# CITlabRostock/citlab-article-separation-new

Measured on AMD Instinct MI355X. Metric: newspaper pages/sec (ARU-Net seg + GNN relation) at 3000x4500 px, higher is better.
Workload: dtype f32s

## Files before the change

citlab-article-separation-new_amd/csrc/res8ws_kernels.h:

```cpp
#pragma once
#include "res8w_kernels.h"
#include "split_kernels.h"

namespace asep {

struct Res8WSProb {
    const float* skip;
    const float* dec;
    const float* img;
    const float* stats;
    float* out;
    float* pool;
    int H, W;
    int n_strips;
    int band;
    int y_end;
    int tile_begin;
};
struct Res8WSArgs {
    Res8WSProb p[MAXP];
    int nprob;
    const float* b1;
    const u32x4* w1s;
    const float* w1f;
    const u32x4* ws;
    const float* bias;
    XcdMap xm;
};

__device__ __forceinline__ void r8ws_mm6(const u32x4 (&w)[3], const u32x4 (&xa)[3], const u32x4 (&xb)[3], f32x4& ca, f32x4& cb) {
    ca = mfma_bf16_k32(w[2], xa[0], ca); cb = mfma_bf16_k32(w[2], xb[0], cb);
    ca = mfma_bf16_k32(w[0], xa[2], ca); cb = mfma_bf16_k32(w[0], xb[2], cb);
    ca = mfma_bf16_k32(w[1], xa[1], ca); cb = mfma_bf16_k32(w[1], xb[1], cb);
    ca = mfma_bf16_k32(w[1], xa[0], ca); cb = mfma_bf16_k32(w[1], xb[0], cb);
    ca = mfma_bf16_k32(w[0], xa[1], ca); cb = mfma_bf16_k32(w[0], xb[1], cb);
    ca = mfma_bf16_k32(w[0], xa[0], ca); cb = mfma_bf16_k32(w[0], xb[0], cb);
}
__device__ __forceinline__ void r8ws_split4(f32x4 v, u32x2& h, u32x2& m, u32x2& l) {
    unsigned h0, m0, l0, h1, m1, l1;
    split3_pair(v.x, v.y, h0, m0, l0);
    split3_pair(v.z, v.w, h1, m1, l1);
    h = u32x2{h0, h1}; m = u32x2{m0, m1}; l = u32x2{l0, l1};
}

template <bool UP>
__global__ __launch_bounds__(64, 1) void res8ws_kernel(const Res8WSArgs a) {
    constexpr int TW = R8W_TW;
    constexpr int W0 = TW + 6, W1 = TW + 4, W2 = TW + 2;
    constexpr int NR = 4, NT = 16;
    constexpr int PL0 = W0 * 16, PL1 = W1 * 16, PL2 = W2 * 16;
    constexpr int IMB = UP ? 0 : 4 * 32 * 4;
    constexpr int R0_OFF = IMB, R1_OFF = R0_OFF + NR * 3 * PL0, R2_OFF = R1_OFF + NR * 3 * PL1, TC_OFF = R2_OFF + NR * 3 * PL2,
                  TRASH = TC_OFF + NT * TW * 32, LDSB = TRASH + 16;
    static_assert(LDSB <= 30 * 1024, "four waves per CU with room to spare");
    __shared__ __attribute__((aligned(16))) unsigned char lds[LDSB];

    const int lane = threadIdx.x;
    const int j = lane & 15, kk = lane >> 4, e = kk >> 1, ch = (kk & 1) * 4;
    const int isB = kk & 1;
    const int c = 2 * j + e;
    const int item = sched_tile(a.xm);
    if (item < 0) return;
    const int pi = prob_of_tile(a, item);
    const Res8WSProb& P = a.p[pi];
    const int li = item - P.tile_begin;
    const int bi = li / P.n_strips, si = li - bi * P.n_strips;
    const int x0 = R8W_X0 + TW * si;
    const int Ya = R8W_Y0 + bi * P.band;
    const int nb = min(P.band, P.y_end - Ya);
    const int W = P.W;

    constexpr int NF1 = UP ? 18 : 0, NFW = 27;
    u32x4 wf[NFW], w1[UP ? NF1 : 1];
    {
        const u32x4* wl = a.ws + lane;
#pragma unroll
        for (int i = 0; i < NFW; ++i) asm volatile("global_load_dwordx4 %0, %1, off" : "=a"(wf[i]) : "v"(wl + i * 64) : "memory");
        if constexpr (UP) {
            const u32x4* w1l = a.w1s + lane;
#pragma unroll
            for (int i = 0; i < NF1; ++i) asm volatile("global_load_dwordx4 %0, %1, off" : "=a"(w1[i]) : "v"(w1l + i * 64) : "memory");
        }
        asm volatile("s_waitcnt vmcnt(0)" ::: "memory");
#pragma unroll
        for (int i = 0; i < NFW; ++i) asm volatile("" : "+a"(wf[i]));
        if constexpr (UP) {
#pragma unroll
            for (int i = 0; i < NF1; ++i) asm volatile("" : "+a"(w1[i]));
        }
    }
    auto wpart = [&](int s, int ky, u32x4 (&o)[3]) {
#pragma unroll
        for (int p = 0; p < 3; ++p) o[p] = wf[(s * 3 + ky) * 3 + p];
    };
    const f32x4 bias1 = *reinterpret_cast<const f32x4*>(a.b1 + ch);
    f32x4 biasw[3];
#pragma unroll
    for (int t = 0; t < 3; ++t) biasw[t] = *reinterpret_cast<const f32x4*>(a.bias + 8 * t + ch);

    const int gxw = min(x0 - 4 + 2 * j + kk, W - 1);
    const float* __restrict__ skp = P.skip;
    const float* __restrict__ dcp = P.dec;
    auto in_row = [&](const float* __restrict__ src, int gy, f32x4& lo, f32x4& hi) {
        const float* q = src + ((size_t)gy * (size_t)W + (size_t)gxw) * 8;
        lo = *reinterpret_cast<const f32x4*>(q);
        hi = *reinterpret_cast<const f32x4*>(q + 4);
    };
    float mean = 0.f, inv = 1.f;
    if constexpr (!UP) {
        if (P.stats) { mean = P.stats[0]; inv = P.stats[1]; }
    }
    const float* __restrict__ imp = P.img;
    const size_t ioff0 = (size_t)(Ya - 4 + (lane >> 5)) * (size_t)W + (size_t)(x0 - 4 + (lane & 31));
    auto iload = [&](int p) { return imp[ioff0 + (size_t)p * 2 * (size_t)W]; };
    float* const iring = reinterpret_cast<float*>(lds);
    auto istore = [&](float v, int p) { iring[(p & 1) * 64 + lane] = (v - mean) * inv; };
    float w1v[UP ? 1 : 36];
    if constexpr (!UP) {
#pragma unroll
        for (int t = 0; t < 9; ++t)
#pragma unroll
            for (int o = 0; o < 4; ++o) w1v[t * 4 + o] = a.w1f[t * 8 + ch + o];
    }

    const int p_last = nb / 2 + 3;
    u32x4 cin[2][2][3] = {};
    f32x4 nxt[2][2][2];
    float inx = 0.f;
    if constexpr (UP) {
#pragma unroll
        for (int r = 0; r < 2; ++r) {
            f32x4 lo, hi;
            in_row(skp, Ya - 4 + r, lo, hi);
            split3_x8(lo, hi, cin[r][0][0], cin[r][0][1], cin[r][0][2]);
            in_row(dcp, Ya - 4 + r, lo, hi);
            split3_x8(lo, hi, cin[r][1][0], cin[r][1][1], cin[r][1][2]);
            in_row(skp, Ya - 2 + r, nxt[r][0][0], nxt[r][0][1]);
            in_row(dcp, Ya - 2 + r, nxt[r][1][0], nxt[r][1][1]);
        }
    } else {
        istore(iload(0), 0);
        inx = iload(1);
    }

    const int lcol = r8w_swz(2 * j + kk) * 16;
    auto whole = [&](u32x2 pa, u32x2 pb) {
        const auto s0 = __builtin_amdgcn_permlane16_swap(pa.x, pb.x, false, false);
        const auto s1 = __builtin_amdgcn_permlane16_swap(pa.y, pb.y, false, false);
        return u32x4{s0[0], s1[0], s0[1], s1[1]};
    };
    const int cs = r8w_swz(c) * 16;
    const bool v0 = j < W0 / 2, v1 = j < W1 / 2, v2 = j < W2 / 2;
    const bool tvalid = c >= 3 && c < 3 + TW;
    const int tcol = (tvalid ? c - 3 : 0) * 32 + ch * 4;
    const int trd = min(c, TW - 1) * 32 + ch * 4;
    const bool ost = j < TW / 2;
    float* __restrict__ const outp = P.out;
    float* __restrict__ const poolp = P.pool;
    const size_t Wp = (size_t)((W + 1) >> 1);

    auto store_parts = [&](f32x4 ra, f32x4 rb, int roff, int pl, bool valid, int rowa, int rowb) {
        u32x2 ha, ma, la, hb, mb, lb;
        r8ws_split4(relu4i(ra), ha, ma, la);
        r8ws_split4(relu4i(rb), hb, mb, lb);
        const u32x4 ph = whole(ha, hb), pm = whole(ma, mb), pl_ = whole(la, lb);
        const int rr = isB ? rowb : rowa;
        const int base = valid ? roff + rr * 3 * pl + cs : TRASH;
        const int step = valid ? pl : 0;
        *reinterpret_cast<u32x4*>(lds + base) = ph;
        *reinterpret_cast<u32x4*>(lds + base + step) = pm;
        *reinterpret_cast<u32x4*>(lds + base + 2 * step) = pl_;
    };
    auto ring_read = [&](int roff, int pl, int rr, u32x4 (&o)[3]) {
#pragma unroll
        for (int p = 0; p < 3; ++p) o[p] = *reinterpret_cast<const u32x4*>(lds + roff + (rr * 3 + p) * pl + lcol);
    };

    const int K = nb / 2 + 6;
#pragma unroll 1
    for (int k = 0; k < K; ++k) {
        const int i4 = (2 * k) & (NR - 1), i16 = (2 * k) & (NT - 1);
        const bool do_c1 = k < nb / 2 + 3, do_s1 = k >= 2 && k < nb / 2 + 4, do_s2 = k >= 4 && k < nb / 2 + 5, do_s3 = k >= 6;

        if (do_s3) {
            u32x4 q[4][3];
#pragma unroll
            for (int r = 0; r < 4; ++r) ring_read(R2_OFF, PL2, (i4 + r - 9) & (NR - 1), q[r]);
            const f32x4 t0 = *reinterpret_cast<const f32x4*>(lds + TC_OFF + ((i16 - 8) & (NT - 1)) * TW * 32 + trd);
            const f32x4 t1 = *reinterpret_cast<const f32x4*>(lds + TC_OFF + ((i16 - 7) & (NT - 1)) * TW * 32 + trd);
            f32x4 va = biasw[2], vb = biasw[2];
#pragma unroll
            for (int ky = 0; ky < 3; ++ky) {
                u32x4 w[3];
                wpart(2, ky, w);
                r8ws_mm6(w, q[ky], q[ky + 1], va, vb);
            }
            va = relu4i(va + t0);
            vb = relu4i(vb + t1);
            const int oy = Ya - 12 + 2 * k;
            if (ost) {
                float* o = outp + ((size_t)oy * (size_t)W + (size_t)(x0 + c)) * 8 + ch;
                *reinterpret_cast<f32x4*>(o) = va;
                *reinterpret_cast<f32x4*>(o + (size_t)W * 8) = vb;
            }
            if constexpr (!UP) {
                if (poolp) {
                    const f32x4 mv = f32x4{fmaxf(va.x, vb.x), fmaxf(va.y, vb.y), fmaxf(va.z, vb.z), fmaxf(va.w, vb.w)};
                    float pm[4];
#pragma unroll
                    for (int i = 0; i < 4; ++i) {
                        const unsigned u = __float_as_uint(mv[i]);
                        const auto s = __builtin_amdgcn_permlane32_swap(u, u, false, false);
                        pm[i] = fmaxf(__uint_as_float(s[0]), __uint_as_float(s[1]));
                    }
                    if (ost && e == 0) {
                        float* po = poolp + ((size_t)(oy >> 1) * Wp + (size_t)((x0 >> 1) + j)) * 8 + ch;
                        *reinterpret_cast<f32x4*>(po) = f32x4{pm[0], pm[1], pm[2], pm[3]};
                    }
                }
            }
        }
        if (do_s2) {
            u32x4 q[4][3];
#pragma unroll
            for (int r = 0; r < 4; ++r) ring_read(R1_OFF, PL1, (i4 + r - 6) & (NR - 1), q[r]);
            f32x4 ra = biasw[1], rb = biasw[1];
#pragma unroll
            for (int ky = 0; ky < 3; ++ky) {
                u32x4 w[3];
                wpart(1, ky, w);
                r8ws_mm6(w, q[ky], q[ky + 1], ra, rb);
            }
            store_parts(ra, rb, R2_OFF, PL2, v2, (i4 - 5) & (NR - 1), (i4 - 4) & (NR - 1));
        }
        if (do_s1) {
            u32x4 q[4][3];
#pragma unroll
            for (int r = 0; r < 4; ++r) ring_read(R0_OFF, PL0, (i4 + r - 3) & (NR - 1), q[r]);
            f32x4 ra = biasw[0], rb = biasw[0];
#pragma unroll
            for (int ky = 0; ky < 3; ++ky) {
                u32x4 w[3];
                wpart(0, ky, w);
                r8ws_mm6(w, q[ky], q[ky + 1], ra, rb);
            }
            store_parts(ra, rb, R1_OFF, PL1, v1, (i4 - 2) & (NR - 1), (i4 - 1) & (NR - 1));
        }
        if (do_c1) {
            f32x4 ra = bias1, rb = bias1;
            if constexpr (UP) {
                u32x4 x2[2][2][3];
#pragma unroll
                for (int r = 0; r < 2; ++r)
#pragma unroll
                    for (int s = 0; s < 2; ++s) split3_x8(nxt[r][s][0], nxt[r][s][1], x2[r][s][0], x2[r][s][1], x2[r][s][2]);
                if (k + 2 <= p_last) {
#pragma unroll
                    for (int r = 0; r < 2; ++r) {
                        in_row(skp, Ya + 2 * k + r, nxt[r][0][0], nxt[r][0][1]);
                        in_row(dcp, Ya + 2 * k + r, nxt[r][1][0], nxt[r][1][1]);
                    }
                }
#pragma unroll
                for (int ky = 0; ky < 3; ++ky)
#pragma unroll
                    for (int s = 0; s < 2; ++s) {
                        u32x4 w[3];
#pragma unroll
                        for (int p = 0; p < 3; ++p) w[p] = w1[(ky * 2 + s) * 3 + p];
                        u32x4 xa[3], xb[3];
#pragma unroll
                        for (int p = 0; p < 3; ++p) {
                            xa[p] = ky == 0 ? cin[0][s][p] : (ky == 1 ? cin[1][s][p] : x2[0][s][p]);
                            xb[p] = ky == 0 ? cin[1][s][p] : (ky == 1 ? x2[0][s][p] : x2[1][s][p]);
                        }
                        r8ws_mm6(w, xa, xb, ra, rb);
                    }
#pragma unroll
                for (int r = 0; r < 2; ++r)
#pragma unroll
                    for (int s = 0; s < 2; ++s)
#pragma unroll
                        for (int p = 0; p < 3; ++p) cin[r][s][p] = x2[r][s][p];
            } else {
                istore(inx, k + 1);
                if (k + 2 <= p_last) inx = iload(k + 2);
                const int cb = min(c, 29);
#pragma unroll
                for (int ky = 0; ky < 3; ++ky)
#pragma unroll
                    for (int kx = 0; kx < 3; ++kx) {
                        const float va = iring[((2 * k + ky) & 3) * 32 + cb + kx], vb = iring[((2 * k + 1 + ky) & 3) * 32 + cb + kx];
#pragma unroll
                        for (int o = 0; o < 4; ++o) {
                            ra[o] = fmaf(va, w1v[(ky * 3 + kx) * 4 + o], ra[o]);
                            rb[o] = fmaf(vb, w1v[(ky * 3 + kx) * 4 + o], rb[o]);
                        }
                    }
            }
            if (tvalid) {
                *reinterpret_cast<f32x4*>(lds + TC_OFF + ((i16 + 1) & (NT - 1)) * TW * 32 + tcol) = ra;
                *reinterpret_cast<f32x4*>(lds + TC_OFF + ((i16 + 2) & (NT - 1)) * TW * 32 + tcol) = rb;
            }
            store_parts(ra, rb, R0_OFF, PL0, v0, (i4 + 1) & (NR - 1), (i4 + 2) & (NR - 1));
        }
    }
}

}
```

Baseline: 151.7.

## Restructure res8ws loop into unrolled steady-state steps with interleaved stages

The row loop moves into a step lambda. The steady-state loop body is unrolled by two with compile-time ring indices and stage predicates, and the conv stages are reordered so MFMA work of one stage overlaps LDS stores of another. The single LDS buffer is split into separate fixed-pitch ring arrays with per-ring trash slots, which drops the per-width plane pitches and the valid-based trash redirection. The DOWN variant raises its launch bound to two waves per SIMD. This adds register pressure and code size, and the padded 32-column rings use slightly more LDS.

Measured after the change: 150.0. 1.1% lower.

```diff
diff --git a/citlab-article-separation-new_amd/csrc/res8ws_kernels.h b/citlab-article-separation-new_amd/csrc/res8ws_kernels.h
--- a/citlab-article-separation-new_amd/csrc/res8ws_kernels.h
+++ b/citlab-article-separation-new_amd/csrc/res8ws_kernels.h
@@ -44,16 +44,15 @@
 }
 
 template <bool UP>
-__global__ __launch_bounds__(64, 1) void res8ws_kernel(const Res8WSArgs a) {
+__global__ __launch_bounds__(64, UP ? 1 : 2) void res8ws_kernel(const Res8WSArgs a) {
     constexpr int TW = R8W_TW;
-    constexpr int W0 = TW + 6, W1 = TW + 4, W2 = TW + 2;
     constexpr int NR = 4, NT = 16;
-    constexpr int PL0 = W0 * 16, PL1 = W1 * 16, PL2 = W2 * 16;
-    constexpr int IMB = UP ? 0 : 4 * 32 * 4;
-    constexpr int R0_OFF = IMB, R1_OFF = R0_OFF + NR * 3 * PL0, R2_OFF = R1_OFF + NR * 3 * PL1, TC_OFF = R2_OFF + NR * 3 * PL2,
-                  TRASH = TC_OFF + NT * TW * 32, LDSB = TRASH + 16;
-    static_assert(LDSB <= 30 * 1024, "four waves per CU with room to spare");
-    __shared__ __attribute__((aligned(16))) unsigned char lds[LDSB];
+    constexpr int PL = 32 * 16, ROW = 3 * PL;
+    constexpr int RINGB = NR * ROW + 64;
+    constexpr int TCB = NT * TW * 32;
+    __shared__ __attribute__((aligned(16))) unsigned char r0s[RINGB], r1s[RINGB], r2s[RINGB], tcs[TCB + 32];
+    __shared__ __attribute__((aligned(16))) float iring[UP ? 4 : 4 * 32];
+    static_assert(3 * RINGB + TCB + 32 + 4 * 32 * 4 <= 31 * 1024, "five waves per CU (DOWN)");
 
     const int lane = threadIdx.x;
     const int j = lane & 15, kk = lane >> 4, e = kk >> 1, ch = (kk & 1) * 4;
@@ -89,10 +88,6 @@
             for (int i = 0; i < NF1; ++i) asm volatile("" : "+a"(w1[i]));
         }
     }
-    auto wpart = [&](int s, int ky, u32x4 (&o)[3]) {
-#pragma unroll
-        for (int p = 0; p < 3; ++p) o[p] = wf[(s * 3 + ky) * 3 + p];
-    };
     const f32x4 bias1 = *reinterpret_cast<const f32x4*>(a.b1 + ch);
     f32x4 biasw[3];
 #pragma unroll
@@ -113,8 +108,7 @@
     const float* __restrict__ imp = P.img;
     const size_t ioff0 = (size_t)(Ya - 4 + (lane >> 5)) * (size_t)W + (size_t)(x0 - 4 + (lane & 31));
     auto iload = [&](int p) { return imp[ioff0 + (size_t)p * 2 * (size_t)W]; };
-    float* const iring = reinterpret_cast<float*>(lds);
-    auto istore = [&](float v, int p) { iring[(p & 1) * 64 + lane] = (v - mean) * inv; };
+    auto istore = [&](float v, int par) { iring[par * 64 + lane] = (v - mean) * inv; };
     float w1v[UP ? 1 : 36];
     if constexpr (!UP) {
 #pragma unroll
@@ -150,53 +144,120 @@
         return u32x4{s0[0], s1[0], s0[1], s1[1]};
     };
     const int cs = r8w_swz(c) * 16;
-    const bool v0 = j < W0 / 2, v1 = j < W1 / 2, v2 = j < W2 / 2;
     const bool tvalid = c >= 3 && c < 3 + TW;
-    const int tcol = (tvalid ? c - 3 : 0) * 32 + ch * 4;
+    const int tcol = (c - 3) * 32 + ch * 4;
     const int trd = min(c, TW - 1) * 32 + ch * 4;
     const bool ost = j < TW / 2;
     float* __restrict__ const outp = P.out;
     float* __restrict__ const poolp = P.pool;
     const size_t Wp = (size_t)((W + 1) >> 1);
 
-    auto store_parts = [&](f32x4 ra, f32x4 rb, int roff, int pl, bool valid, int rowa, int rowb) {
+    auto store_parts = [&](f32x4 ra, f32x4 rb, unsigned char* ring, int rowa, int rowb) {
         u32x2 ha, ma, la, hb, mb, lb;
         r8ws_split4(relu4i(ra), ha, ma, la);
         r8ws_split4(relu4i(rb), hb, mb, lb);
         const u32x4 ph = whole(ha, hb), pm = whole(ma, mb), pl_ = whole(la, lb);
-        const int rr = isB ? rowb : rowa;
-        const int base = valid ? roff + rr * 3 * pl + cs : TRASH;
-        const int step = valid ? pl : 0;
-        *reinterpret_cast<u32x4*>(lds + base) = ph;
-        *reinterpret_cast<u32x4*>(lds + base + step) = pm;
-        *reinterpret_cast<u32x4*>(lds + base + 2 * step) = pl_;
-    };
-    auto ring_read = [&](int roff, int pl, int rr, u32x4 (&o)[3]) {
-#pragma unroll
-        for (int p = 0; p < 3; ++p) o[p] = *reinterpret_cast<const u32x4*>(lds + roff + (rr * 3 + p) * pl + lcol);
-    };
-
-    const int K = nb / 2 + 6;
-#pragma unroll 1
-    for (int k = 0; k < K; ++k) {
-        const int i4 = (2 * k) & (NR - 1), i16 = (2 * k) & (NT - 1);
-        const bool do_c1 = k < nb / 2 + 3, do_s1 = k >= 2 && k < nb / 2 + 4, do_s2 = k >= 4 && k < nb / 2 + 5, do_s3 = k >= 6;
-
+        unsigned char* d = ring + cs + (isB ? rowb : rowa) * ROW;
+        *reinterpret_cast<u32x4*>(d) = ph;
+        *reinterpret_cast<u32x4*>(d + PL) = pm;
+        *reinterpret_cast<u32x4*>(d + 2 * PL) = pl_;
+    };
+    auto ring_read = [&](const unsigned char* ring, int rr, u32x4 (&o)[3]) {
+#pragma unroll
+        for (int p = 0; p < 3; ++p) o[p] = *reinterpret_cast<const u32x4*>(ring + rr * ROW + p * PL + lcol);
+    };
+    auto tail_mm = [&](const unsigned char* ring, int rr0, int s, f32x4& ra, f32x4& rb) {
+        u32x4 q[4][3];
+#pragma unroll
+        for (int r = 0; r < 4; ++r) ring_read(ring, (rr0 + r) & (NR - 1), q[r]);
+#pragma unroll
+        for (int ky = 0; ky < 3; ++ky) {
+            u32x4 w[3];
+#pragma unroll
+            for (int p = 0; p < 3; ++p) w[p] = wf[(s * 3 + ky) * 3 + p];
+            r8ws_mm6(w, q[ky], q[ky + 1], ra, rb);
+        }
+    };
+
+    auto step = [&](auto i4_, int k, auto c1_, auto s1_, auto s2_, auto s3_, auto ld_) __attribute__((always_inline)) {
+        const int i4 = i4_;
+        const bool do_c1 = c1_, do_s1 = s1_, do_s2 = s2_, do_s3 = s3_, do_ld = ld_;
+        const int i16 = (2 * k) & (NT - 1);
+        f32x4 va = biasw[2], vb = biasw[2], t0{}, t1{};
         if (do_s3) {
-            u32x4 q[4][3];
-#pragma unroll
-            for (int r = 0; r < 4; ++r) ring_read(R2_OFF, PL2, (i4 + r - 9) & (NR - 1), q[r]);
-            const f32x4 t0 = *reinterpret_cast<const f32x4*>(lds + TC_OFF + ((i16 - 8) & (NT - 1)) * TW * 32 + trd);
-            const f32x4 t1 = *reinterpret_cast<const f32x4*>(lds + TC_OFF + ((i16 - 7) & (NT - 1)) * TW * 32 + trd);
-            f32x4 va = biasw[2], vb = biasw[2];
-#pragma unroll
-            for (int ky = 0; ky < 3; ++ky) {
-                u32x4 w[3];
-                wpart(2, ky, w);
-                r8ws_mm6(w, q[ky], q[ky + 1], va, vb);
-            }
+            t0 = *reinterpret_cast<const f32x4*>(tcs + ((i16 - 8) & (NT - 1)) * TW * 32 + trd);
+            t1 = *reinterpret_cast<const f32x4*>(tcs + ((i16 - 7) & (NT - 1)) * TW * 32 + trd);
+            tail_mm(r2s, i4 - 9, 2, va, vb);
+        }
+        f32x4 r2a = biasw[1], r2b = biasw[1];
+        if (do_s2) tail_mm(r1s, i4 - 6, 1, r2a, r2b);
+        if (do_s3) {
             va = relu4i(va + t0);
             vb = relu4i(vb + t1);
+        }
+        f32x4 r1a = biasw[0], r1b = biasw[0];
+        if (do_s1) tail_mm(r0s, i4 - 3, 0, r1a, r1b);
+        if (do_s2) store_parts(r2a, r2b, r2s, (i4 - 5) & (NR - 1), (i4 - 4) & (NR - 1));
+        f32x4 ra = bias1, rb = bias1;
+        if (do_c1) {
+            if constexpr (UP) {
+                u32x4 x2[2][2][3];
+#pragma unroll
+                for (int r = 0; r < 2; ++r)
+#pragma unroll
+                    for (int s = 0; s < 2; ++s) split3_x8(nxt[r][s][0], nxt[r][s][1], x2[r][s][0], x2[r][s][1], x2[r][s][2]);
+                if (do_ld) {
+#pragma unroll
+                    for (int r = 0; r < 2; ++r) {
+                        in_row(skp, Ya + 2 * k + r, nxt[r][0][0], nxt[r][0][1]);
+                        in_row(dcp, Ya + 2 * k + r, nxt[r][1][0], nxt[r][1][1]);
+                    }
+                }
+#pragma unroll
+                for (int ky = 0; ky < 3; ++ky)
+#pragma unroll
+                    for (int s = 0; s < 2; ++s) {
+                        u32x4 w[3];
+#pragma unroll
+                        for (int p = 0; p < 3; ++p) w[p] = w1[(ky * 2 + s) * 3 + p];
+                        u32x4 xa[3], xb[3];
+#pragma unroll
+                        for (int p = 0; p < 3; ++p) {
+                            xa[p] = ky == 0 ? cin[0][s][p] : (ky == 1 ? cin[1][s][p] : x2[0][s][p]);
+                            xb[p] = ky == 0 ? cin[1][s][p] : (ky == 1 ? x2[0][s][p] : x2[1][s][p]);
+                        }
+                        r8ws_mm6(w, xa, xb, ra, rb);
+                    }
+#pragma unroll
+                for (int r = 0; r < 2; ++r)
+#pragma unroll
+                    for (int s = 0; s < 2; ++s)
+#pragma unroll
+                        for (int p = 0; p < 3; ++p) cin[r][s][p] = x2[r][s][p];
+            } else {
+                istore(inx, ((i4 >> 1) + 1) & 1);
+                if (do_ld) inx = iload(k + 2);
+                const int cb = min(c, 29);
+#pragma unroll
+                for (int ky = 0; ky < 3; ++ky)
+#pragma unroll
+                    for (int kx = 0; kx < 3; ++kx) {
+                        const float xa = iring[((i4 + ky) & 3) * 32 + cb + kx], xb = iring[((i4 + 1 + ky) & 3) * 32 + cb + kx];
+#pragma unroll
+                        for (int o = 0; o < 4; ++o) {
+                            ra[o] = fmaf(xa, w1v[(ky * 3 + kx) * 4 + o], ra[o]);
+                            rb[o] = fmaf(xb, w1v[(ky * 3 + kx) * 4 + o], rb[o]);
+                        }
+                    }
+            }
+        }
+        if (do_s1) store_parts(r1a, r1b, r1s, (i4 - 2) & (NR - 1), (i4 - 1) & (NR - 1));
+        if (do_c1) {
+            *reinterpret_cast<f32x4*>(tcs + (tvalid ? ((i16 + 1) & (NT - 1)) * TW * 32 + tcol : TCB)) = ra;
+            *reinterpret_cast<f32x4*>(tcs + (tvalid ? ((i16 + 2) & (NT - 1)) * TW * 32 + tcol : TCB + 16)) = rb;
+            store_parts(ra, rb, r0s, (i4 + 1) & (NR - 1), (i4 + 2) & (NR - 1));
+        }
+        if (do_s3) {
             const int oy = Ya - 12 + 2 * k;
             if (ost) {
                 float* o = outp + ((size_t)oy * (size_t)W + (size_t)(x0 + c)) * 8 + ch;
@@ -220,89 +281,21 @@
                 }
             }
         }
-        if (do_s2) {
-            u32x4 q[4][3];
-#pragma unroll
-            for (int r = 0; r < 4; ++r) ring_read(R1_OFF, PL1, (i4 + r - 6) & (NR - 1), q[r]);
-            f32x4 ra = biasw[1], rb = biasw[1];
-#pragma unroll
-            for (int ky = 0; ky < 3; ++ky) {
-                u32x4 w[3];
-                wpart(1, ky, w);
-                r8ws_mm6(w, q[ky], q[ky + 1], ra, rb);
-            }
-            store_parts(ra, rb, R2_OFF, PL2, v2, (i4 - 5) & (NR - 1), (i4 - 4) & (NR - 1));
-        }
-        if (do_s1) {
-            u32x4 q[4][3];
-#pragma unroll
-            for (int r = 0; r < 4; ++r) ring_read(R0_OFF, PL0, (i4 + r - 3) & (NR - 1), q[r]);
-            f32x4 ra = biasw[0], rb = biasw[0];
-#pragma unroll
-            for (int ky = 0; ky < 3; ++ky) {
-                u32x4 w[3];
-                wpart(0, ky, w);
-                r8ws_mm6(w, q[ky], q[ky + 1], ra, rb);
-            }
-            store_parts(ra, rb, R1_OFF, PL1, v1, (i4 - 2) & (NR - 1), (i4 - 1) & (NR - 1));
-        }
-        if (do_c1) {
-            f32x4 ra = bias1, rb = bias1;
-            if constexpr (UP) {
-                u32x4 x2[2][2][3];
-#pragma unroll
-                for (int r = 0; r < 2; ++r)
-#pragma unroll
-                    for (int s = 0; s < 2; ++s) split3_x8(nxt[r][s][0], nxt[r][s][1], x2[r][s][0], x2[r][s][1], x2[r][s][2]);
-                if (k + 2 <= p_last) {
-#pragma unroll
-                    for (int r = 0; r < 2; ++r) {
-                        in_row(skp, Ya + 2 * k + r, nxt[r][0][0], nxt[r][0][1]);
-                        in_row(dcp, Ya + 2 * k + r, nxt[r][1][0], nxt[r][1][1]);
-                    }
-                }
-#pragma unroll
-                for (int ky = 0; ky < 3; ++ky)
-#pragma unroll
-                    for (int s = 0; s < 2; ++s) {
-                        u32x4 w[3];
-#pragma unroll
-                        for (int p = 0; p < 3; ++p) w[p] = w1[(ky * 2 + s) * 3 + p];
-                        u32x4 xa[3], xb[3];
-#pragma unroll
-                        for (int p = 0; p < 3; ++p) {
-                            xa[p] = ky == 0 ? cin[0][s][p] : (ky == 1 ? cin[1][s][p] : x2[0][s][p]);
-                            xb[p] = ky == 0 ? cin[1][s][p] : (ky == 1 ? x2[0][s][p] : x2[1][s][p]);
-                        }
-                        r8ws_mm6(w, xa, xb, ra, rb);
-                    }
-#pragma unroll
-                for (int r = 0; r < 2; ++r)
-#pragma unroll
-                    for (int s = 0; s < 2; ++s)
-#pragma unroll
-                        for (int p = 0; p < 3; ++p) cin[r][s][p] = x2[r][s][p];
-            } else {
-                istore(inx, k + 1);
-                if (k + 2 <= p_last) inx = iload(k + 2);
-                const int cb = min(c, 29);
-#pragma unroll
-                for (int ky = 0; ky < 3; ++ky)
-#pragma unroll
-                    for (int kx = 0; kx < 3; ++kx) {
-                        const float va = iring[((2 * k + ky) & 3) * 32 + cb + kx], vb = iring[((2 * k + 1 + ky) & 3) * 32 + cb + kx];
-#pragma unroll
-                        for (int o = 0; o < 4; ++o) {
-                            ra[o] = fmaf(va, w1v[(ky * 3 + kx) * 4 + o], ra[o]);
-                            rb[o] = fmaf(vb, w1v[(ky * 3 + kx) * 4 + o], rb[o]);
-                        }
-                    }
-            }
-            if (tvalid) {
-                *reinterpret_cast<f32x4*>(lds + TC_OFF + ((i16 + 1) & (NT - 1)) * TW * 32 + tcol) = ra;
-                *reinterpret_cast<f32x4*>(lds + TC_OFF + ((i16 + 2) & (NT - 1)) * TW * 32 + tcol) = rb;
-            }
-            store_parts(ra, rb, R0_OFF, PL0, v0, (i4 + 1) & (NR - 1), (i4 + 2) & (NR - 1));
+    };
+
+    const int K = nb / 2 + 6, ks = nb / 2 + 2;
+    using C0 = std::integral_constant<int, 0>;
+    using C2 = std::integral_constant<int, 2>;
+    constexpr std::true_type on{};
+    int k = 0;
+    while (k < K) {
+        if (k >= 6 && k + 1 < ks) {
+            step(C0{}, k, on, on, on, on, on);
+            step(C2{}, k + 1, on, on, on, on, on);
+            k += 2;
+        } else {
+            step((2 * k) & (NR - 1), k, k < nb / 2 + 3, k >= 2 && k < nb / 2 + 4, k >= 4 && k < nb / 2 + 5, k >= 6, k + 2 <= p_last);
+            ++k;
         }
     }
 }
```
